# awslabs/flowgger

Hardware: NVIDIA H100
Metric: log lines/sec parsed (RFC5424) (higher is better)
Workload: dtype u8

## Files before the change

### flowgger_b200/csrc/fg_abi.cu

```cuda
#include <cuda_runtime.h>

#include <algorithm>
#include <chrono>
#include <cstdio>
#include <cstdlib>
#include <cstring>
#include <ctime>
#include <mutex>
#include <new>
#include <string>
#include <utility>
#include <vector>

#include "../../include/flowgger_cuda.h"
#include "fg_kernels.cuh"
#include "fg_status.h"
#include "fg_rfc3164.cuh"
#include "fg_tz.h"

namespace {

const char* kErrorStrings[FG_ST_COUNT] = {};
struct ErrorTableInit {
    ErrorTableInit() {
// ... 89 lines not shown
struct Handle {
    H h = nullptr;
    Handle() = default;
    Handle(Handle&& o) noexcept : h(o.h) { o.h = nullptr; }
    Handle(const Handle&) = delete;
    Handle& operator=(const Handle&) = delete;
    ~Handle() {
        if (h) destroy(h);
    }
    operator H() const { return h; }
};
using Event = Handle<cudaEvent_t>;
using Stream = Handle<cudaStream_t>;

struct StepEvents {
    Event h2d;
    Event k0, k1;
    Event cnt;
};

enum { T_ENTRIES, T_E8, T_ARENA, T_WIDE, T_COUNT };
struct TableShape {
    size_t width[3];
    size_t round;
};
constexpr TableShape kTableShape[T_COUNT] = {
    {{sizeof(fg_span), sizeof(uint64_t), 1}, 256},
    {{sizeof(uint64_t), 0, 0}, 256},
    {{1, 0, 0}, 256},
    {{sizeof(fg_wide_row), 0, 0}, 1},
};
static_assert(sizeof(fg_span) == sizeof(int2) && sizeof(fg_wide_row) == sizeof(fg::WideRow), "pinned rows mirror the device rows");
struct Table {
    Buf<uint8_t> col[3];
    size_t cap = 0;
};

struct TableUse {
    int table, counter;
    size_t div, floor;
    bool grow;
};
struct FormatTables {
    int n;
    TableUse use[4];
    const TableUse* begin() const { return use; }
    const TableUse* end() const { return use + n; }
};
constexpr FormatTables kFormatTables[4] = {
    {4, {{T_E8, fg::K5_ENTRIES, 24, 4096, false}, {T_ARENA, fg::K5_ARENA, 64, 64 << 10, false},
         {T_WIDE, fg::K5_WIDE_ROWS, 0, 1024, false}, {T_ENTRIES, fg::K5_WIDE_ENTRIES, 0, 4096, false}}},
    {1, {{T_ENTRIES, fg::K5_ENTRIES, 24, 4096, true}}},
    {1, {{T_ENTRIES, fg::K5_ENTRIES, 24, 4096, true}}},
    {2, {{T_ARENA, fg::K5_ARENA, 32, 64 << 10, false}, {T_ENTRIES, -1, 0, 256, false}}},
};

}

struct fg_ctx {
    int device = 0;
    size_t max_bytes = 0;
    int max_lines = 0;
    int chunk_lines = 0;
    Stream s_h2d, s_comp, s_d2h;
    Stream s_parse;
    Event ev_a, ev_b;
    Event ev_dom0, ev_dom1;
    Event ev_s0, ev_s1;
    std::vector<StepEvents> steps;
    std::vector<Event> ev_split;
    Event bounce_ev[2];
    Buf<uint8_t> bounce[2];
    Buf<uint32_t> counts;
    Buf<uint8_t> bytes;
    Buf<int32_t> offsets;
    Buf<uint32_t> k;
    Buf<uint8_t> flush;
    Table tab[T_COUNT];
    Buf<uint8_t> rows;
    Buf<int2> tmp_name;
    Buf<unsigned long long> tmp_val;
    Buf<uint8_t> tmp_meta;
    Buf<fg::Row5424, fg_row5424> rows5;
    Buf<uint32_t> esc_list, wide_list;
    Buf<uint32_t> enc_lens, enc_rel;
    Buf<unsigned long long> enc_base;
    Buf<uint8_t> enc_out;
    size_t enc_out_cap = 0;
    Buf<long long, int64_t> enc_offsets;
    Buf<uint8_t> enc_status;
    Buf<uint8_t> scan_temp;
    size_t scan_temp_bytes = 0;
    Buf<uint8_t> static_blob;
    int n_static = 0;
    const int32_t* d_static_key_off = nullptr;
    const int32_t* d_static_lit_off = nullptr;
    const int32_t* d_static_kind = nullptr;
    std::vector<std::pair<std::string, std::string>> gelf_extra;
    Buf<uint32_t> seg;
    Buf<int32_t> n_lines;
    Buf<uint8_t> invalid;
    Buf<int32_t> split_offsets;
    Buf<int32_t> cum;
    float last_split_ms = 0.f;
    int r3164_year = 0;
    int call_year = 1970;
    std::string tzdir;
    fg::TzHostTable tz_host;
    Buf<uint8_t> tz_blob;
    fg::TzDeviceTable tz_dev{};
    Buf<uint8_t> ltsv_blob;
    fg::LtsvDeviceConfig ltsv{};
    float last_dom_ms = 0.f;
    int res_n = 0;
    size_t res_bytes = 0;
    int res_fmt = -1;
    uint32_t res_tot[fg::K5_COUNT] = {};
    std::string last_error;
    int64_t launches = 0;
    int max_tile5 = 0;
    int num_sms = 0;
};

namespace {

constexpr int kColW[9] = {8, 4, 8, 8, 8, 8, 8, 8, 8};
enum { C_TS = 0, C_META, C_HOST, C_APP, C_PROC, C_MSGID, C_MSG, C_FULL, C_SD, C_COUNT };
size_t col_off(const fg_ctx* c, int col) {
    const size_t n = (size_t)c->max_lines;
    size_t o = 0;
    for (int k = 0; k < col; ++k) o += (size_t)kColW[k] * n;
    return o;
}

int fail(fg_ctx* c, int code, const char* what, cudaError_t e = cudaSuccess) {
    if (c) {
        c->last_error = what;
        if (e != cudaSuccess) {
            c->last_error += ": ";
            c->last_error += cudaGetErrorString(e);
        }
    }
    return code;
}

#define FG_CUDA(ctx, call)                                         \
    do {                                                           \
        cudaError_t _e = (call);                                   \
        if (_e != cudaSuccess) return fail(ctx, FG_E_CUDA, #call, _e); \
    } while (0)

cudaError_t create(Event& e, unsigned flags) { return cudaEventCreateWithFlags(&e.h, flags); }
cudaError_t create(Stream& s) { return cudaStreamCreateWithFlags(&s.h, cudaStreamNonBlocking); }

template <class T>
T* dev(const fg_ctx* c, int t, int col = 0) {
    return reinterpret_cast<T*>(c->tab[t].col[col].d);
}
template <class T>
T* host(const fg_ctx* c, int t, int col = 0) {
    return reinterpret_cast<T*>(c->tab[t].col[col].h);
}
uint32_t cap32(const fg_ctx* c, int t) { return (uint32_t)std::min<size_t>(c->tab[t].cap, 0xFFFFFFFFu); }

int grow_table(fg_ctx* c, int t, size_t rows) {
    const TableShape& S = kTableShape[t];
    Table& T = c->tab[t];
// ... 36 lines not shown
    std::vector<uint8_t> bytes;
    template <class V>
    size_t add(const V& v) {
        const size_t at = bytes.size();
        const uint8_t* src = reinterpret_cast<const uint8_t*>(v.data());
        bytes.insert(bytes.end(), src, src + v.size() * sizeof(v[0]));
        bytes.resize((bytes.size() + 15) & ~(size_t)15, 0);
        return at;
    }
    int upload(fg_ctx* c, Buf<uint8_t>& blob) {
        bytes.resize(bytes.size() + 16, 0);
        FG_CUDA(c, blob.alloc(bytes.size(), DEV));
        FG_CUDA(c, cudaMemcpy(blob.d, bytes.data(), bytes.size(), cudaMemcpyHostToDevice));
        return FG_OK;
    }
};

int upload_tz(fg_ctx* c) {
    const fg::TzHostTable& H = c->tz_host;
    Packer p;
    const size_t o_hash = p.add(H.hash), o_key = p.add(H.key), o_zone = p.add(H.zone), o_noff = p.add(H.name_off),
                 o_first = p.add(H.first), o_off = p.add(H.off), o_names = p.add(H.names);
    if (int rc = p.upload(c, c->tz_blob)) return rc;
    const uint8_t* b = c->tz_blob.d;
    fg::TzDeviceTable& T = c->tz_dev;
    T = H.view();
    T.hash = (const unsigned long long*)(b + o_hash);
    T.key = (const long long*)(b + o_key);
    T.zone = (const int32_t*)(b + o_zone);
    T.name_off = (const int32_t*)(b + o_noff);
    T.first = (const int32_t*)(b + o_first);
    T.off = (const int32_t*)(b + o_off);
    T.names = b + o_names;
    return FG_OK;
}

int upload_ltsv_config(fg_ctx* c, const fg_config* cfg) {
    std::vector<uint8_t> names, suffix;
    std::vector<int32_t> name_off{0}, types;
    const int ns = (cfg->ltsv_schema_names && cfg->ltsv_schema_types) ? cfg->ltsv_schema_len : 0;
    for (int k = 0; k < ns; ++k) {
        const char* s = cfg->ltsv_schema_names[k];
        names.insert(names.end(), (const uint8_t*)s, (const uint8_t*)s + strlen(s));
        name_off.push_back((int32_t)names.size());
        types.push_back(cfg->ltsv_schema_types[k]);
    }
    fg::LtsvDeviceConfig& L = c->ltsv;
    L.has_schema = (cfg->ltsv_has_schema || ns > 0) ? 1 : 0;
    L.n_schema = ns;
    L.suffix_present = 0;
    L.suffix_off[0] = 0;
    for (int t = 0; t < 5; ++t) {
        const char* s = cfg->ltsv_suffix[t];
        if (t > 0 && s) {
            L.suffix_present |= 1u << t;
            suffix.insert(suffix.end(), (const uint8_t*)s, (const uint8_t*)s + strlen(s));
        }
        L.suffix_off[t + 1] = (int32_t)suffix.size();
    }
    Packer p;
    const size_t o_names = p.add(names), o_off = p.add(name_off), o_types = p.add(types), o_suf = p.add(suffix);
    if (int rc = p.upload(c, c->ltsv_blob)) return rc;
    const uint8_t* b = c->ltsv_blob.d;
    L.names = b + o_names;
    L.name_off = (const int32_t*)(b + o_off);
    L.types = (const int32_t*)(b + o_types);
    L.suffix = b + o_suf;
    return FG_OK;
}

int current_year(const fg_ctx* c) {
    if (c->r3164_year != 0) return c->r3164_year;
    const time_t now = time(nullptr);
    struct tm g;
    gmtime_r(&now, &g);
    return g.tm_year + 1900;
}

int ensure_format(fg_ctx* c, int fmt) {
    const size_t L = (size_t)c->max_lines;
    if (fmt == FG_FMT_RFC5424) {
        if (!c->rows5.d) {
            FG_CUDA(c, c->rows5.alloc(L, BOTH));
            FG_CUDA(c, c->esc_list.alloc(L, DEV));
            FG_CUDA(c, c->wide_list.alloc(L, DEV));
        }
    } else if (!c->rows.d) {
        FG_CUDA(c, c->rows.alloc(col_off(c, C_COUNT), BOTH));
    }
    if (fmt == FG_FMT_GELF && !c->wide_list.d) FG_CUDA(c, c->wide_list.alloc(L, DEV));
    for (const TableUse& u : kFormatTables[fmt]) {
        const size_t first = u.div ? std::max<size_t>(c->max_bytes / u.div, u.floor) : u.floor;
        const size_t cap = c->tab[u.table].cap;
        if (u.grow ? cap < first : !cap)
            if (int rc = grow_table(c, u.table, first)) return rc;
    }
    if (fmt == FG_FMT_RFC3164) {
        if (!c->tz_host.loaded) {
            std::string err;
            if (!fg::tz_load_dir(c->tzdir.empty() ? nullptr : c->tzdir.c_str(), c->tz_host, err)) return fail(c, FG_E_ARG, err.c_str());
        }
        if (!c->tz_blob.d)
            if (int rc = upload_tz(c)) return rc;
    }
    if (fmt == FG_FMT_LTSV || fmt == FG_FMT_GELF) {
        const size_t need = (fmt == FG_FMT_LTSV ? c->max_bytes / 2 + L : c->max_bytes / 3) + 64;
        if (c->tmp_meta.n < need) {
            c->tmp_name.reset(); c->tmp_val.reset(); c->tmp_meta.reset();
            FG_CUDA(c, c->tmp_name.alloc(need, DEV));
            FG_CUDA(c, c->tmp_val.alloc(need, DEV));
            FG_CUDA(c, c->tmp_meta.alloc(need, DEV));
        }
    }
    return FG_OK;
}

int begin_call(fg_ctx* c, fg_format fmt) {
    if ((int)fmt < 0 || (int)fmt > 3) return fail(c, FG_E_ARG, "unknown format");
    FG_CUDA(c, cudaSetDevice(c->device));
    if (int rc = ensure_format(c, (int)fmt)) return rc;
    c->call_year = current_year(c);
    return FG_OK;
}

int pick_tile(const fg_ctx* c, size_t total_bytes, int n, int fmt) {
    const double mean = n > 0 ? (double)total_bytes / n : 0.0;
    const long lines = fg::lines_per_cta(fmt), gran = 8 * lines;
    const int max_tile[4] = {c->max_tile5, fg::kLtsvMaxTile, fg::kGelfMaxTile, fg::kR3164MaxTile};
    long t = (long)(mean * lines * 1.02) + gran;
    t = (t + gran - 1) / gran * gran;
    t = std::max(t, 8L * 1024);
    t = std::min(t, (long)max_tile[fmt]);
    return (int)t;
}

int launch_lines(fg_ctx* c, int fmt, int line0, int n, int tile, const uint8_t* invalid, int strip_eol, cudaStream_t s,
                 bool time_dominant = false) {
    if (fmt == FG_FMT_RFC5424) {
        fg::Parse5424Params P;
        P.bytes = c->bytes.d;
        P.offsets = c->offsets.d + line0;
        P.n = n;
        P.tile_bytes = tile;
        P.rows = reinterpret_cast<uint4*>(c->rows5.d + line0);
        P.entries = dev<unsigned long long>(c, T_E8);
        P.entry_cap = cap32(c, T_E8);
        P.counters = c->k.d;
        P.esc_list = c->esc_list.d;
        P.wide_list = c->wide_list.d;
        P.arena = dev<uint8_t>(c, T_ARENA);
        P.arena_cap = cap32(c, T_ARENA);
        P.wide_rows = dev<fg::WideRow>(c, T_WIDE);
        P.wide_cap = cap32(c, T_WIDE);
        P.wentry_name = dev<int2>(c, T_ENTRIES, 0);
        P.wentry_val = dev<unsigned long long>(c, T_ENTRIES, 1);
        P.wentry_meta = dev<uint8_t>(c, T_ENTRIES, 2);
        P.wentry_cap = cap32(c, T_ENTRIES);
        P.line0 = line0;
        P.bad_offsets = c->k.d + fg::K5_BAD_OFFSETS;
        P.line_invalid = invalid;
        P.strip_eol = strip_eol;
        P.num_sms = c->num_sms;
        FG_CUDA(c, cudaMemsetAsync(c->k.d + fg::K5_ESC_LIST, 0, 8, s));
        FG_CUDA(c, fg::launch_parse5424(P, s, time_dominant ? c->ev_dom0.h : nullptr, time_dominant ? c->ev_dom1.h : nullptr));
        c->launches += 2;
        return FG_OK;
    }
    fg::ParseParams P;
    P.bytes = c->bytes.d;
    P.offsets = c->offsets.d + line0;
    P.n = n;
    P.line0 = line0;
    P.tile_bytes = tile;
    P.num_sms = c->num_sms;
    uint8_t* r = c->rows.d;
    P.ts = (double*)(r + col_off(c, C_TS)) + line0;
    P.meta = (uint32_t*)(r + col_off(c, C_META)) + line0;
    P.host = (int2*)(r + col_off(c, C_HOST)) + line0;
    P.app = (int2*)(r + col_off(c, C_APP)) + line0;
    P.proc = (int2*)(r + col_off(c, C_PROC)) + line0;
    P.msgid = (int2*)(r + col_off(c, C_MSGID)) + line0;
    P.msg = (int2*)(r + col_off(c, C_MSG)) + line0;
    P.full = (int2*)(r + col_off(c, C_FULL)) + line0;
    P.sd = (int2*)(r + col_off(c, C_SD)) + line0;
    P.entry_name = dev<int2>(c, T_ENTRIES, 0);
    P.entry_val = dev<unsigned long long>(c, T_ENTRIES, 1);
    P.entry_meta = dev<uint8_t>(c, T_ENTRIES, 2);
    P.tmp_name = c->tmp_name.d;
    P.tmp_val = c->tmp_val.d;
    P.tmp_meta = c->tmp_meta.d;
    P.line_invalid = invalid;
    P.strip_eol = strip_eol;
    P.entry_counter = c->k.d + fg::K5_ENTRIES;
    P.entry_cap = cap32(c, T_ENTRIES);
    P.bad_offsets = c->k.d + fg::K5_BAD_OFFSETS;
    P.slow_list = c->wide_list.d;
    P.slow_count = c->k.d + fg::K5_WIDE_LIST;
    if (fmt == FG_FMT_GELF) FG_CUDA(c, cudaMemsetAsync(c->k.d + fg::K5_WIDE_LIST, 0, 4, s));
    P.ltsv = c->ltsv;
    P.r3164.year = c->call_year;
    P.r3164.tz = c->tz_dev;
    P.r3164.arena = dev<uint8_t>(c, T_ARENA);
    P.r3164.arena_cap = cap32(c, T_ARENA);
    P.r3164.arena_counter = c->k.d + fg::K5_ARENA;
    if (time_dominant) FG_CUDA(c, cudaEventRecord(c->ev_dom0, s));
    FG_CUDA(c, fg::launch_parse(fmt, P, s));
    if (time_dominant) FG_CUDA(c, cudaEventRecord(c->ev_dom1, s));
    c->launches += fmt == FG_FMT_GELF ? 2 : 1;
    return FG_OK;
}

int launch_encode(fg_ctx* c, int k, int l0, int n, int tile, cudaStream_t s) {
    fg::GelfEncodeParams E;
    E.bytes = c->bytes.d;
    E.offsets = c->offsets.d + l0;
    E.n = n;
    E.rows = reinterpret_cast<const uint4*>(c->rows5.d + l0);
    E.entries = dev<unsigned long long>(c, T_E8);
    E.arena = dev<uint8_t>(c, T_ARENA);
    E.wide_rows = dev<fg::WideRow>(c, T_WIDE);
    E.wentry_name = dev<int2>(c, T_ENTRIES, 0);
    E.wentry_val = dev<unsigned long long>(c, T_ENTRIES, 1);
    E.wentry_meta = dev<uint8_t>(c, T_ENTRIES, 2);
    E.static_blob = c->static_blob.d;
    E.n_static = c->n_static;
    E.static_key_off = c->d_static_key_off;
    E.static_lit_off = c->d_static_lit_off;
    E.static_kind = c->d_static_kind;
    E.lens = c->enc_lens.d + l0;
    E.rel = c->enc_rel.d + l0;
    E.base = c->enc_base.d + k;
    E.out = c->enc_out.d;
    E.out_cap = c->enc_out_cap;
    E.out_offsets = c->enc_offsets.d + l0;
    E.status = c->enc_status.d + l0;
    E.bad_offsets = c->k.d + fg::K5_BAD_OFFSETS;
    E.entry_cap = cap32(c, T_E8);
    E.wide_cap = cap32(c, T_WIDE);
    E.wentry_cap = cap32(c, T_ENTRIES);
    E.tile_bytes = std::min(4 * tile, c->max_tile5);
    FG_CUDA(c, fg::launch_gelf_encode(E, c->scan_temp.d, c->scan_temp_bytes, s));
    c->launches += 4;
    return FG_OK;
}

bool col_used(int col) { return !(col == C_APP || col == C_PROC || col == C_MSGID); }
// ... 754 lines not shown
```

### flowgger_b200/csrc/fg_kernels.cuh

```cuda
#pragma once
#include <stdint.h>
#ifdef FG_HOST_EMU
#include "../../tests/emu/cuda_shim.h"
#else
#include <cuda_runtime.h>
#endif

namespace fg {

struct LtsvDeviceConfig {
    int32_t has_schema;
    int32_t n_schema;
    const uint8_t* names;
    const int32_t* name_off;
    const int32_t* types;
    const uint8_t* suffix;
    int32_t suffix_off[6];
    uint32_t suffix_present;
};

struct TzDeviceTable {
    int32_t n_names;
    int32_t min_len, max_len;
    uint32_t first_mask[8];
    const unsigned long long* hash;
    const int32_t* zone;
    const int32_t* name_off;
    const uint8_t* names;
    const int32_t* first;
    const long long* key;
    const int32_t* off;
};
struct R3164DeviceConfig {
    int32_t year;
    TzDeviceTable tz;
    uint8_t* arena;
    uint32_t arena_cap;
    uint32_t* arena_counter;
};

struct ParseParams {
    const uint8_t* bytes;
    const int32_t* offsets;
    int32_t n;
    int32_t line0;
    int32_t tile_bytes;
    double* ts;
    uint32_t* meta;
    int2* host;
    int2* app;
    int2* proc;
    int2* msgid;
    int2* msg;
    int2* full;
    int2* sd;
    int2* entry_name;
    unsigned long long* entry_val;
    uint8_t* entry_meta;
    int2* tmp_name;
    unsigned long long* tmp_val;
    uint8_t* tmp_meta;
    const uint8_t* line_invalid;
    int32_t strip_eol;
    uint32_t* entry_counter;
    uint32_t entry_cap;
    const uint32_t* bad_offsets;
    uint32_t* slow_list;
    uint32_t* slow_count;
    int32_t num_sms;
    LtsvDeviceConfig ltsv;
    R3164DeviceConfig r3164;
};

struct Row5424 {
    double ts;
    uint32_t meta;
    uint32_t sd_first;
    uint16_t sd_count;
    uint16_t sp[5];
    uint16_t msg_off, msg_len;
};
static_assert(sizeof(Row5424) == 32, "Row5424 must be 32 bytes");
struct WideRow {
    int32_t line;
    uint32_t meta;
    double ts;
    int2 host, app, proc, msgid, msg, full, sd;
};
static_assert(sizeof(WideRow) == 72, "WideRow must be 72 bytes");

enum { K5_ENTRIES = 0, K5_ARENA = 1, K5_WIDE_ROWS = 2, K5_WIDE_ENTRIES = 3, K5_ESC_LIST = 4, K5_WIDE_LIST = 5, K5_BAD_OFFSETS = 6,
       K5_COUNT = 8 };

struct Parse5424Params {
    const uint8_t* bytes;
    const int32_t* offsets;
    int32_t n;
    int32_t tile_bytes;
    uint4* rows;
    unsigned long long* entries;
    uint32_t entry_cap;
    uint32_t* counters;
    uint32_t* esc_list;
    uint32_t* wide_list;
    uint8_t* arena;
    uint32_t arena_cap;
    WideRow* wide_rows;
    uint32_t wide_cap;
    int2* wentry_name;
    unsigned long long* wentry_val;
    uint8_t* wentry_meta;
    uint32_t wentry_cap;
    int32_t line0;
    const uint32_t* bad_offsets;
    const uint8_t* line_invalid;
    int32_t strip_eol;
    int32_t num_sms;
};

cudaError_t launch_parse5424(const Parse5424Params& p, cudaStream_t stream, cudaEvent_t dom0 = nullptr, cudaEvent_t dom1 = nullptr);
cudaError_t configure_parse5424(int max_tile_bytes);
int parse5424_smem_bytes(int tile_bytes);

struct GelfEncodeParams {
    const uint8_t* bytes;
    const int32_t* offsets;
    int32_t n;
    const uint4* rows;
    const unsigned long long* entries;
    const uint8_t* arena;
    const WideRow* wide_rows;
    const int2* wentry_name;
    const unsigned long long* wentry_val;
    const uint8_t* wentry_meta;
    const uint8_t* static_blob;
    int32_t n_static;
    const int32_t* static_key_off;
    const int32_t* static_lit_off;
    const int32_t* static_kind;
    uint32_t* lens;
    uint32_t* rel;
    unsigned long long* base;
    uint8_t* out;
    unsigned long long out_cap;
    long long* out_offsets;
    uint8_t* status;
    const uint32_t* bad_offsets;
    uint32_t entry_cap, wide_cap, wentry_cap;
    int32_t tile_bytes;
};
cudaError_t configure_gelf_encode(int max_tile_bytes);
cudaError_t launch_gelf_encode(const GelfEncodeParams& p, void* d_scan_temp, size_t scan_temp_bytes, cudaStream_t stream);
size_t gelf_scan_temp_bytes(int n);

#ifndef FG_R5_LINES
#define FG_R5_LINES 64
#endif
#ifndef FG_R5_MINB
#define FG_R5_MINB 16
#endif
constexpr int kRfc5424LinesPerCta = FG_R5_LINES;
constexpr int kRfc5424CtasPerSm = FG_R5_MINB;
#ifndef FG_LTSV_LINES
#define FG_LTSV_LINES 64
#endif
#ifndef FG_LTSV_THREADS
#define FG_LTSV_THREADS 256
#endif
constexpr int kLtsvLinesPerCta = FG_LTSV_LINES;
constexpr int kLtsvThreadsPerCta = FG_LTSV_THREADS;
constexpr int kLtsvStageSlots = kLtsvLinesPerCta * 24;
constexpr int kLtsvMaxTile = 65024;
#ifndef FG_GELF_LINES
#define FG_GELF_LINES 64
#endif
#ifndef FG_GELF_THREADS
#define FG_GELF_THREADS 256
#endif
constexpr int kGelfLinesPerCta = FG_GELF_LINES;
constexpr int kGelfThreadsPerCta = FG_GELF_THREADS;
constexpr int kGelfCtasPerSm = 3;
constexpr int kGelfStageSlots = kGelfLinesPerCta * 16;
constexpr int kGelfMaxTile = 65024;
#ifndef FG_R3_LINES
#define FG_R3_LINES 64
#endif
// ... 33 lines not shown
```

### flowgger_b200/csrc/fg_parse5424.cu

```cuda
#include "fg_kernels.cuh"

#include "fg_common.cuh"
#include "fg_r5fast.cuh"
#include "fg_rfc5424.cuh"
#include "fg_status.h"
#include "fg_tma.cuh"

namespace fg {

namespace {

constexpr int kFastLines = kRfc5424LinesPerCta;
constexpr int kFastCtasPerSm = kRfc5424CtasPerSm;

template <int LINES, int MINB>
__global__ void __launch_bounds__(LINES, MINB) parse5424_kernel(const __grid_constant__ Parse5424Params P) {
    extern __shared__ __align__(128) uint8_t tile[];
    __shared__ __align__(8) uint64_t mbar;
    __shared__ uint32_t scan_ws[2 * (LINES / 32)];
    __shared__ uint32_t s_base[3];

    const int tid = threadIdx.x;
    const uint32_t lane = (uint32_t)tid & 31u;
    const int first = blockIdx.x * LINES;
    const int last = min(P.n, first + LINES);
    uint32_t* bmI = reinterpret_cast<uint32_t*>(tile + P.tile_bytes);
    if (*P.bad_offsets) return;
    if (tid == 0) mbar_init(&mbar, 1);
    __syncthreads();

    uint32_t parity = 0;
    int cur = first;
    while (cur < last) {
        const int i = cur + tid;
        const int o0 = __ldg(P.offsets + min(i, last));
        const int o1 = __ldg(P.offsets + min(i + 1, last));
        const int ocur = __ldg(P.offsets + cur);
        const int base = ocur & ~15;
        const bool fits = (i < last) && (o1 - base <= P.tile_bytes);
        const int r = __syncthreads_count(fits);
        if (r == 0) {
            if (tid == 0) P.wide_list[atomicAdd(P.counters + K5_WIDE_LIST, 1u)] = (uint32_t)cur;
            cur += 1;
            continue;
        }
        const int oend = __ldg(P.offsets + cur + r);
        const uint32_t nbytes = (uint32_t)((oend - base) + 15) & ~15u;
        if (tid == 0) {
            fence_proxy_async();
            mbar_expect_tx(&mbar, nbytes);
            bulk_g2s(tile, P.bytes + base, nbytes, &mbar);
        }
        mbar_wait(&mbar, parity);
        parity ^= 1u;

        const int nword = (int)((nbytes + 31u) >> 5);
        for (int g = tid; g < nword; g += LINES) {
            const uint4 v0 = reinterpret_cast<const uint4*>(tile)[2 * g], v1 = reinterpret_cast<const uint4*>(tile)[2 * g + 1];
            bmI[g] = r5_classify16(v0.x, v0.y, v0.z, v0.w) | (r5_classify16(v1.x, v1.y, v1.z, v1.w) << 16);
        }
        if (tid < 3) bmI[nword + tid] = 0;
        __syncthreads();

        const bool active = tid < r;
        int ls = active ? o0 - base : 0;
        int le = active ? o1 - base : 0;
        bool bad_utf8 = false;
        if (P.strip_eol && le > ls) {
            if (P.strip_eol == 2) {
                if (tile[le - 1] == 0) --le;
            } else if (tile[le - 1] == '\n') {
                --le;
                if (le > ls && tile[le - 1] == '\r') --le;
            }
            if (P.line_invalid != nullptr && P.line_invalid[i]) bad_utf8 = true;
        }
        const bool too_long = le - ls > 65535;
        R5Fast res;
        const bool regular = r5_regular(tile, bmI, ls, (too_long || bad_utf8 || !active) ? ls : le, res);
        if (bad_utf8) {
            res.status = FG_ES_INVALID_UTF8;
            res.n_entries = 0;
        }
        const bool wide = active && !regular && !bad_utf8;
        const uint32_t my_n = (active && !wide && res.status == FG_ST_OK) ? res.n_entries : 0u;
        const bool esc = my_n != 0u && res.esc;

        uint32_t xa = my_n, xb = (esc ? 1u : 0u) | (wide ? 0x100u : 0u);
#pragma unroll
        for (int d = 1; d < 32; d <<= 1) {
            const uint32_t ya = __shfl_up_sync(0xFFFFFFFFu, xa, d), yb = __shfl_up_sync(0xFFFFFFFFu, xb, d);
            if (lane >= (uint32_t)d) { xa += ya; xb += yb; }
        }
        const int wid = tid >> 5;
        constexpr int kWarps = LINES / 32;
        if (lane == 31u) { scan_ws[wid] = xa; scan_ws[kWarps + wid] = xb; }
        __syncthreads();
        uint32_t before_a = 0, before_b = 0, total = 0, total_b = 0;
#pragma unroll
        for (int w = 0; w < kWarps; ++w) {
            const uint32_t ta = scan_ws[w], tb = scan_ws[kWarps + w];
            if (w < wid) { before_a += ta; before_b += tb; }
            total += ta;
            total_b += tb;
        }
        const uint32_t excl = before_a + xa - my_n;
        const uint32_t pos_b = before_b + xb - ((esc ? 1u : 0u) | (wide ? 0x100u : 0u));
        const uint32_t n_esc = total_b & 0xFFu, n_wide = total_b >> 8;
        if (total | total_b) {
            if (tid == 0 && total) s_base[0] = atomicAdd(P.counters + K5_ENTRIES, total);
            if (tid == 32 % LINES && n_esc) s_base[1] = atomicAdd(P.counters + K5_ESC_LIST, n_esc);
            if (tid == 33 % LINES && n_wide) s_base[2] = atomicAdd(P.counters + K5_WIDE_LIST, n_wide);
            __syncthreads();
        }
        const uint32_t esc_at = pos_b & 0xFFu, wide_at = pos_b >> 8;
        uint32_t my_begin = 0;
        if (my_n) {
            my_begin = s_base[0] + excl;
            if ((unsigned long long)my_begin + my_n <= (unsigned long long)P.entry_cap) {
                unsigned long long* dst = P.entries + my_begin;
                for (uint32_t k = 0; k < my_n; ++k) dst[k] = res.stage[k];
            }
        }
        if (esc) P.esc_list[s_base[1] + esc_at] = (uint32_t)i;
        if (wide) P.wide_list[s_base[2] + wide_at] = (uint32_t)i;
        if (active && !wide) {
            const bool ok = res.status == FG_ST_OK;
            const uint32_t meta = ok ? (res.facility << 8) | (res.severity << 16) | (res.flags << 24) : res.status | 0x00FFFF00u;
            uint4 lo4, hi4;
            lo4.x = (uint32_t)__double2loint(res.ts);
            lo4.y = (uint32_t)__double2hiint(res.ts);
            lo4.z = meta;
            lo4.w = my_begin;
            hi4.x = my_n | ((uint32_t)res.sp1 << 16);
            hi4.y = (uint32_t)res.sp2 | ((uint32_t)res.sp3 << 16);
            hi4.z = (uint32_t)res.sp4 | ((uint32_t)res.sp5 << 16);
            hi4.w = (uint32_t)res.msg_o | ((uint32_t)res.msg_l << 16);
            if (!ok) {
                lo4.x = lo4.y = 0u;
                hi4 = make_uint4(0u, 0u, 0u, 0u);
            }
            P.rows[2 * (size_t)i] = lo4;
            P.rows[2 * (size_t)i + 1] = hi4;
        }
        __syncthreads();
        cur += r;
    }
}

__device__ __forceinline__ void unescape_lines(const Parse5424Params& P, uint32_t first_item, uint32_t stride) {
    const uint32_t cnt = P.counters[K5_ESC_LIST];
    const uint32_t lane = threadIdx.x & 31u;
    for (uint32_t j0 = first_item; j0 < cnt; j0 += stride) {
        const uint32_t j = j0 + lane;
        const bool valid = j < cnt;
        uint32_t first = 0, count = 0;
        int o0 = 0;
        if (valid) {
            const uint32_t line = P.esc_list[j];
            const uint4 lo4 = P.rows[2 * (size_t)line], hi4 = P.rows[2 * (size_t)line + 1];
            o0 = P.offsets[line];
            first = lo4.w;
            count = hi4.x & 0xFFFFu;
            if ((unsigned long long)first + count > (unsigned long long)P.entry_cap) count = 0;
        }
        uint32_t need = 0;
        for (uint32_t e = 0; e < count; ++e) {
            const unsigned long long v = P.entries[first + e];
            if (!(v & kE8Header) && (v & kE8Esc)) need += (2u + (uint32_t)((v >> 32) & 0xFFFFu) - ((uint32_t)((v >> 16) & 0xFFFFu) + 2u) + 1u) & ~1u;
        }
        uint32_t inc = need;
#pragma unroll
        for (int d = 1; d < 32; d <<= 1) {
            const uint32_t y = __shfl_up_sync(0xFFFFFFFFu, inc, d);
            if (lane >= (uint32_t)d) inc += y;
        }
        const uint32_t warp_total = __shfl_sync(0xFFFFFFFFu, inc, 31);
        uint32_t abase = 0;
        if (lane == 0 && warp_total) abase = atomicAdd(P.counters + K5_ARENA, warp_total);
        abase = __shfl_sync(0xFFFFFFFFu, abase, 0);
        if ((unsigned long long)abase + warp_total > (unsigned long long)P.arena_cap) continue;
        uint32_t at = abase + inc - need;
        uint32_t e = 0;
        for (;;) {
            unsigned long long v = 0;
            bool have = false;
            for (; e < count; ++e) {
                v = P.entries[first + e];
                if (!(v & kE8Header) && (v & kE8Esc)) { have = true; break; }
            }
            if (!__any_sync(0xFFFFFFFFu, have)) break;
            const int ne = (int)((v >> 16) & 0xFFFFu), ve = (int)((v >> 32) & 0xFFFFu);
            const int len = have ? ve - (ne + 2) : 0;
            const uint8_t* src = P.bytes + o0 + ne + 2;
            uint8_t* dst = P.arena + at + 2;
            int k = 0, o = 0;
            while (__any_sync(0xFFFFFFFFu, k < len)) {
                if (k < len) {
                    const uint32_t c = src[k++];
                    if (c != '\\') {
                        dst[o++] = (uint8_t)c;
                    } else if (k < len) {
                        const uint32_t d = src[k++];
                        if (d != '"' && d != '\\' && d != ']') dst[o++] = '\\';
                        dst[o++] = (uint8_t)d;
                    }
                }
            }
            if (have) {
                *reinterpret_cast<uint16_t*>(P.arena + at) = (uint16_t)o;
                P.entries[first + e] = (v & 0xFFFFFFFFull) | ((unsigned long long)(at >> 1) << 32) | kE8Arena;
                at += (2u + (uint32_t)len + 1u) & ~1u;
                ++e;
            }
        }
    }
}

__device__ __forceinline__ void wide_lines(const Parse5424Params& P, int (*marks)[32], uint32_t first_item, uint32_t stride) {
    const uint32_t cnt = P.counters[K5_WIDE_LIST];
    const uint32_t lane = threadIdx.x & 31u;
    const EntrySink sink = {P.wentry_name, P.wentry_val, P.wentry_meta};
    for (uint32_t j0 = first_item; j0 < cnt; j0 += stride) {
        const uint32_t j = j0 + lane;
        const bool valid = j < cnt;
        uint32_t line = 0;
        int o0 = 0, len = 0;
        bool bad_utf8 = false;
        if (valid) {
            line = P.wide_list[j];
            o0 = P.offsets[line];
            len = P.offsets[line + 1] - o0;
            if (P.strip_eol && len > 0) {
                if (P.strip_eol == 2) {
                    if (P.bytes[o0 + len - 1] == 0) --len;
                } else if (P.bytes[o0 + len - 1] == '\n') {
                    --len;
                    if (len > 0 && P.bytes[o0 + len - 1] == '\r') --len;
                }
                if (P.line_invalid != nullptr && P.line_invalid[line]) bad_utf8 = true;
            }
            if (bad_utf8) len = 0;
        }
        LineResult res;
        rfc5424_parse_line<32>(P.bytes + o0, len, o0, &marks[0][lane], res, sink, 0u, false);
        uint32_t n = (valid && !bad_utf8 && res.status == FG_ST_OK) ? res.n_entries : 0u;
        uint32_t wbase = 0;
        if (n) {
            wbase = atomicAdd(P.counters + K5_WIDE_ENTRIES, n);
            if ((unsigned long long)wbase + n > (unsigned long long)P.wentry_cap) n = 0;
        }
        {
            LineResult again;
            rfc5424_parse_line<32>(P.bytes + o0, n ? len : 0, o0, &marks[0][lane], again, sink, wbase, true);
        }
        if (!valid) continue;
        for (uint32_t k = 0; k < n; ++k) {
            const uint32_t e = wbase + k;
            const uint8_t m = sink.meta[e];
            if ((m & 0x07u) == 0u && (m & 0x08u)) {
                const unsigned long long v = sink.val[e];
                const uint32_t off = (uint32_t)v, l = (uint32_t)(v >> 32);
                const uint32_t ul = (uint32_t)r5_unescape(P.bytes + off, (int)l, nullptr);
                const uint32_t at = atomicAdd(P.counters + K5_ARENA, (ul + 1u) & ~1u);
                if ((unsigned long long)at + ul <= (unsigned long long)P.arena_cap) r5_unescape(P.bytes + off, (int)l, P.arena + at);
                sink.val[e] = (unsigned long long)at | ((unsigned long long)ul << 32);
                sink.meta[e] = (uint8_t)0x80u;
            }
        }
        if (bad_utf8) {
            res.status = FG_ES_INVALID_UTF8;
            res.flags = 0;
            res.facility = res.severity = 0xFFu;
        }
        const bool ok = res.status == FG_ST_OK;
        if (!ok) {
            P.rows[2 * (size_t)line] = make_uint4(0u, 0u, res.status | 0x00FFFF00u, 0u);
            P.rows[2 * (size_t)line + 1] = make_uint4(0u, 0u, 0u, 0u);
            continue;
        }
        const uint32_t widx = atomicAdd(P.counters + K5_WIDE_ROWS, 1u);
        const uint32_t meta = res.status | (res.facility << 8) | (res.severity << 16) | ((res.flags | kFlagWide) << 24);
        if (widx < P.wide_cap) {
            WideRow w;
            w.line = P.line0 + (int32_t)line;
            w.meta = meta;
            w.ts = res.ts;
            w.host = make_int2(ok ? o0 + res.host_o : -1, res.host_l);
            w.app = make_int2(ok ? o0 + res.app_o : -1, res.app_l);
            w.proc = make_int2(ok ? o0 + res.proc_o : -1, res.proc_l);
            w.msgid = make_int2(ok ? o0 + res.mid_o : -1, res.mid_l);
            w.msg = make_int2(ok && res.msg_o >= 0 ? o0 + res.msg_o : -1, res.msg_l);
            w.full = make_int2(ok && res.full_o >= 0 ? o0 + res.full_o : -1, res.full_l);
            w.sd = make_int2((int)wbase, (int)(ok ? n : 0u));
            P.wide_rows[widx] = w;
        }
        P.rows[2 * (size_t)line] = make_uint4((uint32_t)__double2loint(res.ts), (uint32_t)__double2hiint(res.ts), meta, widx);
        P.rows[2 * (size_t)line + 1] = make_uint4(0u, 0u, 0u, 0u);
    }
}

__global__ void __launch_bounds__(128) post5424_kernel(const __grid_constant__ Parse5424Params P, int esc_ctas) {
    __shared__ int marks[4][6][32];
    if (*P.bad_offsets) return;
    const uint32_t warp = threadIdx.x >> 5;
    if ((int)blockIdx.x < esc_ctas) {
        unescape_lines(P, (blockIdx.x * 4u + warp) * 32u, (uint32_t)esc_ctas * 128u);
    } else {
        const uint32_t wctas = gridDim.x - (uint32_t)esc_ctas;
        wide_lines(P, marks[warp], ((blockIdx.x - (uint32_t)esc_ctas) * 4u + warp) * 32u, wctas * 128u);
    }
}

}

int parse5424_smem_bytes(int tile_bytes) { return tile_bytes + tile_bytes / 8 + 16; }

cudaError_t configure_parse5424(int max_tile_bytes) {
    return cudaFuncSetAttribute(parse5424_kernel<kFastLines, kFastCtasPerSm>, cudaFuncAttributeMaxDynamicSharedMemorySize,
                                parse5424_smem_bytes(max_tile_bytes));
}

cudaError_t launch_parse5424(const Parse5424Params& p, cudaStream_t stream, cudaEvent_t dom0, cudaEvent_t dom1) {
    if (p.n <= 0) return cudaSuccess;
    const int grid = (p.n + kFastLines - 1) / kFastLines;
    if (dom0) cudaEventRecord(dom0, stream);
    parse5424_kernel<kFastLines, kFastCtasPerSm><<<grid, kFastLines, parse5424_smem_bytes(p.tile_bytes), stream>>>(p);
    if (dom1) cudaEventRecord(dom1, stream);
    const long long sms = p.num_sms;
    const int esc_ctas = (int)min((long long)(p.n + 127) / 128, sms * 12);
    const int wide_ctas = (int)min((long long)(p.n + 127) / 128, sms * 4);
    post5424_kernel<<<esc_ctas + wide_ctas, 128, 0, stream>>>(p, esc_ctas);
    return cudaGetLastError();
}

}
```

### flowgger_b200/csrc/fg_r5fast.cuh

```cuda
#pragma once
#include "fg_common.cuh"
#include "fg_status.h"

namespace fg {

FG_DEV uint32_t r5_flags(uint32_t w) {
    const uint32_t low = w & 0x7F7F7F7Fu;
    const uint32_t a2 = low + 0x5D5D5D5Du;
    const uint32_t a1 = low + 0x01010101u;
    const uint32_t x = (w & 0x1E1E1E1Eu) ^ 0x1C1C1C1Cu;
    const uint32_t a3 = x + 0x7F7F7F7Fu;
    return (~a2 | a1 | w | ~a3) & 0x80808080u;
}
FG_DEV uint32_t r5_nibble_top(uint32_t f) { return f * 0x00204081u; }
FG_DEV uint32_t r5_gather16(uint32_t f0, uint32_t f1, uint32_t f2, uint32_t f3) {
    const uint32_t n0 = r5_nibble_top(f0), n1 = r5_nibble_top(f1), n2 = r5_nibble_top(f2), n3 = r5_nibble_top(f3);
    return (n0 >> 28) | ((n1 >> 24) & 0xF0u) | ((n2 >> 20) & 0xF00u) | ((n3 >> 16) & 0xF000u);
}
FG_DEV uint32_t r5_classify16(uint32_t w0, uint32_t w1, uint32_t w2, uint32_t w3) {
    return r5_gather16(r5_flags(w0), r5_flags(w1), r5_flags(w2), r5_flags(w3));
}
FG_DEV uint32_t r5_window(const uint32_t* bm, int t) {
    const int k = t >> 5;
    return fg_funnel_r(bm[k], bm[k + 1], (uint32_t)t & 31u);
}

constexpr unsigned long long kE8Esc = 1ull << 48;
constexpr unsigned long long kE8Header = 1ull << 63;
constexpr unsigned long long kE8Arena = 1ull << 62;
FG_DEV unsigned long long r5_pack_pair8(int ns, int ne, int ve, bool esc) {
    return (unsigned long long)(uint32_t)ns | ((unsigned long long)(uint32_t)ne << 16) | ((unsigned long long)(uint32_t)ve << 32) |
           (esc ? kE8Esc : 0ull);
}
FG_DEV unsigned long long r5_pack_header8(int es, int id_end, uint32_t pairs) {
    return (unsigned long long)(uint32_t)es | ((unsigned long long)(uint32_t)id_end << 16) | ((unsigned long long)(pairs & 0xFFFFu) << 32) | kE8Header;
}

struct R5Fast {
    double ts;
    uint32_t status, facility, severity, flags;
    int sp1, sp2, sp3, sp4, sp5;
    int msg_o, msg_l;
    uint32_t n_entries;
    unsigned long long* stage;
    bool esc;
};

FG_DEV int r5_unescape(const uint8_t* v, int len, uint8_t* out) {
    int o = 0;
    bool esc = false;
    for (int k = 0; k < len; ++k) {
        const uint8_t c = v[k];
        if (!esc) {
            if (c == '\\') esc = true;
            else {
                if (out) out[o] = c;
                ++o;
            }
        } else {
            if (c != '"' && c != '\\' && c != ']') {
                if (out) out[o] = '\\';
                ++o;
            }
            if (out) out[o] = c;
            ++o;
            esc = false;
        }
    }
    return o;
}

FG_DEV int r5_unescape_to(const uint8_t* v, int len, uint8_t* out) {
    int o = 0;
    for (int k = 0; k < len; ++k) {
        const uint32_t c = v[k];
        if (c != '\\') {
            out[o++] = (uint8_t)c;
        } else if (k + 1 < len) {
            const uint32_t d = v[++k];
            if (d != '"' && d != '\\' && d != ']') out[o++] = '\\';
            out[o++] = (uint8_t)d;
        }
    }
    return o;
}

constexpr uint32_t kFlagWide = 0x80u;

FG_DEV uint32_t r5_digit(const uint8_t* T, int at, uint32_t& worst) {
    const uint32_t d = (uint32_t)T[at] - (uint32_t)'0';
    worst = max(worst, d);
    return d;
}

FG_DEV bool r5_regular(uint8_t* T, const uint32_t* bmI, int ls, int le, R5Fast& r) {
    r.ts = 0.0;
    r.status = FG_ST_OK;
    r.facility = 0xFFu;
    r.severity = 0xFFu;
    r.flags = 0;
    r.sp1 = r.sp2 = r.sp3 = r.sp4 = r.sp5 = 0;
    r.msg_o = r.msg_l = 0;
    r.n_entries = 0;
    r.stage = nullptr;
    r.esc = false;
    bool ok = le - ls >= 32;

    int sp[6];
    {
        int t = ls + 1;
#pragma unroll
        for (int k = 0; k < 6; ++k) {
            uint32_t W = r5_window(bmI, t);
            if (k == 1 && W == 0u) {
                t += 32;
                W = r5_window(bmI, t);
            }
            t += fg_ffs(W) - 1;
            ok = ok && W != 0u && t < le && T[t] == ' ';
            sp[k] = t;
            t = ok ? t + 1 : ls;
        }
    }
    uint32_t bad = 0;
    {
        const int l0 = sp[0] - ls;
        ok = ok && T[ls] == '<' && l0 >= 4 && l0 <= 6;
        const int gt = ok ? sp[0] - 2 : ls;
        ok = ok && T[gt] == '>' && T[gt + 1] == '1';
        uint32_t pri = 0;
        for (int q = ls + 1; q < gt; ++q) pri = pri * 10u + r5_digit(T, q, bad);
        ok = ok && pri <= 255u;
        r.facility = pri >> 3;
        r.severity = pri & 7u;
    }
    {
        const int a = ok ? sp[0] + 1 : ls, e = ok ? sp[1] : ls;
        const int L = e - a;
        ok = ok && L >= 20;
        const int z = ok ? e - 1 : ls;
        const bool zulu = T[z] == 'Z';
        const int zone = zulu ? z : z - 5;
        DateTime t;
        t.year = (int)(r5_digit(T, a, bad) * 1000u + r5_digit(T, a + 1, bad) * 100u + r5_digit(T, a + 2, bad) * 10u + r5_digit(T, a + 3, bad));
        t.month = (int)(r5_digit(T, a + 5, bad) * 10u + r5_digit(T, a + 6, bad));
        t.day = (int)(r5_digit(T, a + 8, bad) * 10u + r5_digit(T, a + 9, bad));
        t.hour = (int)(r5_digit(T, a + 11, bad) * 10u + r5_digit(T, a + 12, bad));
        t.minute = (int)(r5_digit(T, a + 14, bad) * 10u + r5_digit(T, a + 15, bad));
        t.second = (int)(r5_digit(T, a + 17, bad) * 10u + r5_digit(T, a + 18, bad));
        ok = ok && T[a + 4] == '-' && T[a + 7] == '-' && T[a + 10] == 'T' && T[a + 13] == ':' && T[a + 16] == ':';
        const int fl = zone - (a + 19);
        ok = ok && (fl == 0 || (fl >= 2 && fl <= 10 && T[a + 19] == '.'));
        uint32_t nanos = 0, mult = 100000000u;
#pragma unroll
        for (int k = 0; k < 9; ++k) {
            if (k + 1 < fl) nanos += r5_digit(T, a + 20 + k, bad) * mult;
            mult /= 10u;
        }
        t.nanos = nanos;
        int off = 0;
        if (!zulu) {
            const uint32_t sg = T[zone];
            const int oh = (int)(r5_digit(T, zone + 1, bad) * 10u + r5_digit(T, zone + 2, bad));
            const int om = (int)(r5_digit(T, zone + 4, bad) * 10u + r5_digit(T, zone + 5, bad));
            ok = ok && (sg == '+' || sg == '-') && T[zone + 3] == ':' && oh <= 23 && om <= 59 && zone >= a + 19;
            off = oh * 3600 + om * 60;
            if (sg == '-') off = -off;
        }
        t.offset_seconds = off;
        ok = ok && bad <= 9u && t.second <= 59;
        if (!ok) { t.year = 2000; t.month = 1; t.day = 1; t.hour = t.minute = t.second = 0; t.nanos = 0; t.offset_seconds = 0; }
        double ts = 0.0;
        ok = finish_datetime(t, false, ts) && ok;
        r.ts = ts;
    }
    fg_syncwarp();

    const int d = ok ? sp[5] + 1 : ls;
    int msg_from = le;
    bool walk = false;
    ok = ok && d < le;
    if (ok) {
        const uint32_t c0 = T[d];
        if (c0 == '-') msg_from = d + 1;
        else if (c0 == '[') walk = true;
        else ok = false;
    }
    {
        const int sbase = (ls + 7) & ~7;
        unsigned long long* stg = (unsigned long long*)(T + sbase);
        uint32_t n = 0, pairs = 0, hdr = 0;
        int i = d + 1, elem_start = 0, id_end = 0;
        bool st_id = true, active = walk, any_esc = false;
        while (fg_any(active)) {
            if (active && st_id) {
                const uint32_t W = r5_window(bmI, i);
                const int s1 = i + fg_ffs(W) - 1;
                if (W == 0u || s1 >= le || T[s1] != ' ') { ok = false; active = false; }
                else { elem_start = i; id_end = s1; i = s1 + 1; st_id = false; hdr = n++; pairs = 0; }
            }
            int e = i;
            if (active) {
                const uint32_t W = r5_window(bmI, i);
                e = i + fg_ffs(W) - 1;
                if (W == 0u || (W & 1u) || e + 2 >= le || T[e] != '=' || T[e + 1] != '"') { ok = false; active = false; }
            }
            int c = e + 2;
            bool has_bs = false;
            {
                bool s = active;
                for (;;) {
                    if (s) {
                        uint32_t W = r5_window(bmI, c);
                        const int room = le - c;
                        if (room < 32) W &= (1u << room) - 1u;
                        int adv = 32;
                        while (W) {
                            const int b = fg_ffs(W) - 1;
                            const uint32_t ch = T[c + b];
                            if (ch == '"') { adv = b; s = false; break; }
                            W &= W - 1u;
                            if (ch == '\\') {
                                has_bs = true;
                                W &= ~(2u << b);
                                if (b == 31) adv = 33;
                            }
                        }
                        c += adv;
                        if (s && c >= le) { c = le; s = false; }
                    }
                    if (!fg_any(s)) break;
                }
            }
            if (active) {
                if (c + 1 >= le || sbase + 8 * ((int)n + 1) > c + 1) { ok = false; active = false; }
                else {
                    stg[n++] = r5_pack_pair8(i - ls, e - ls, c - ls, has_bs);
                    any_esc |= has_bs;
                    ++pairs;
                    const uint32_t nx = T[c + 1];
                    if (nx == ' ') {
                        i = c + 2;
                        if (i >= le) { ok = false; active = false; }
                    } else if (nx == ']') {
                        stg[hdr] = r5_pack_header8(elem_start - ls, id_end - ls, pairs);
                        const uint32_t n2 = c + 2 < le ? T[c + 2] : 0u;
                        if (n2 == ' ') { msg_from = c + 2; active = false; }
                        else if (n2 == '[') { i = c + 3; st_id = true; }
                        else { ok = false; active = false; }
                    } else { ok = false; active = false; }
                }
            }
        }
        if (walk && ok) {
            r.n_entries = n;
            r.stage = stg;
            r.esc = any_esc;
        }
    }

    int hi = le, lo = msg_from;
    {
        bool plain_end = true, plain_start = true;
        if (ok) {
            const uint32_t cl = T[le - 1];
            plain_end = cl > 0x20u && cl < 0x80u;
            plain_start = false;
            if (msg_from + 1 < le) {
                const uint32_t c0 = T[msg_from], c1 = T[msg_from + 1];
                plain_start = c0 == ' ' && c1 > 0x20u && c1 < 0x80u;
            }
        }
        if (fg_any(!plain_end)) {
            if (ok && !plain_end) hi = trim_end(T, msg_from, le);
        }
        if (fg_any(!plain_start)) {
            if (ok) lo = plain_start ? msg_from + 1 : trim_start(T, msg_from, hi);
        } else {
            lo = msg_from + 1;
        }
    }
    if (ok) {
        if (hi > lo) {
            r.msg_o = lo - ls;
            r.msg_l = hi - lo;
        } else {
            r.msg_o = msg_from - ls;
            r.msg_l = 0;
        }
        r.sp1 = sp[1] - ls;
        r.sp2 = sp[2] - ls;
        r.sp3 = sp[3] - ls;
        r.sp4 = sp[4] - ls;
        r.sp5 = sp[5] - ls;
    }
    fg_syncwarp();
    return ok;
}

}
```

Measured before the change: 6.730 billion.

## Fuse structured-data unescaping into RFC5424 parse kernel, drop esc_list post pass

Moves the unescaping of backslash-escaped structured-data values out of the separate post5424 pass and into the main parse kernel. Each line now computes its arena byte need while walking the SD section, a warp scan reserves arena space in a single atomic per block, and a warp-cooperative ballot-based unescaper writes values straight from the shared tile or global bytes. This removes the esc_list buffer, one counter reset, the extra post-kernel CTAs, and the re-reads of rows and entries from global memory. In exchange the parse kernel gains extra registers and warp-synchronous loops, which may reduce occupancy on the main hot path.

```diff
diff --git a/flowgger_b200/csrc/fg_abi.cu b/flowgger_b200/csrc/fg_abi.cu
--- a/flowgger_b200/csrc/fg_abi.cu
+++ b/flowgger_b200/csrc/fg_abi.cu
@@ -195,7 +195,7 @@
     Buf<unsigned long long> tmp_val;
     Buf<uint8_t> tmp_meta;
     Buf<fg::Row5424, fg_row5424> rows5;
-    Buf<uint32_t> esc_list, wide_list;
+    Buf<uint32_t> wide_list;
     Buf<uint32_t> enc_lens, enc_rel;
     Buf<unsigned long long> enc_base;
     Buf<uint8_t> enc_out;
@@ -398,7 +398,6 @@
     if (fmt == FG_FMT_RFC5424) {
         if (!c->rows5.d) {
             FG_CUDA(c, c->rows5.alloc(L, BOTH));
-            FG_CUDA(c, c->esc_list.alloc(L, DEV));
             FG_CUDA(c, c->wide_list.alloc(L, DEV));
         }
     } else if (!c->rows.d) {
@@ -462,7 +461,6 @@
         P.entries = dev<unsigned long long>(c, T_E8);
         P.entry_cap = cap32(c, T_E8);
         P.counters = c->k.d;
-        P.esc_list = c->esc_list.d;
         P.wide_list = c->wide_list.d;
         P.arena = dev<uint8_t>(c, T_ARENA);
         P.arena_cap = cap32(c, T_ARENA);
@@ -477,7 +475,7 @@
         P.line_invalid = invalid;
         P.strip_eol = strip_eol;
         P.num_sms = c->num_sms;
-        FG_CUDA(c, cudaMemsetAsync(c->k.d + fg::K5_ESC_LIST, 0, 8, s));
+        FG_CUDA(c, cudaMemsetAsync(c->k.d + fg::K5_WIDE_LIST, 0, 4, s));
         FG_CUDA(c, fg::launch_parse5424(P, s, time_dominant ? c->ev_dom0.h : nullptr, time_dominant ? c->ev_dom1.h : nullptr));
         c->launches += 2;
         return FG_OK;
diff --git a/flowgger_b200/csrc/fg_kernels.cuh b/flowgger_b200/csrc/fg_kernels.cuh
--- a/flowgger_b200/csrc/fg_kernels.cuh
+++ b/flowgger_b200/csrc/fg_kernels.cuh
@@ -89,8 +89,7 @@
 };
 static_assert(sizeof(WideRow) == 72, "WideRow must be 72 bytes");
 
-enum { K5_ENTRIES = 0, K5_ARENA = 1, K5_WIDE_ROWS = 2, K5_WIDE_ENTRIES = 3, K5_ESC_LIST = 4, K5_WIDE_LIST = 5, K5_BAD_OFFSETS = 6,
-       K5_COUNT = 8 };
+enum { K5_ENTRIES = 0, K5_ARENA = 1, K5_WIDE_ROWS = 2, K5_WIDE_ENTRIES = 3, K5_WIDE_LIST = 5, K5_BAD_OFFSETS = 6, K5_COUNT = 8 };
 
 struct Parse5424Params {
     const uint8_t* bytes;
@@ -101,7 +100,6 @@
     unsigned long long* entries;
     uint32_t entry_cap;
     uint32_t* counters;
-    uint32_t* esc_list;
     uint32_t* wide_list;
     uint8_t* arena;
     uint32_t arena_cap;
diff --git a/flowgger_b200/csrc/fg_parse5424.cu b/flowgger_b200/csrc/fg_parse5424.cu
--- a/flowgger_b200/csrc/fg_parse5424.cu
+++ b/flowgger_b200/csrc/fg_parse5424.cu
@@ -12,6 +12,21 @@
 
 constexpr int kFastLines = kRfc5424LinesPerCta;
 constexpr int kFastCtasPerSm = kRfc5424CtasPerSm;
+
+__device__ __forceinline__ int unescape_warp(const uint8_t* src, int len, uint8_t* out, uint32_t lane) {
+    uint32_t carry = 0;
+    int o = 0;
+    for (int c0 = 0; c0 < len; c0 += 32) {
+        const int j = c0 + (int)lane;
+        const uint32_t b = j < len ? src[j] : 0u, nb = j + 1 < len ? src[j + 1] : 0u;
+        const uint32_t bs = __ballot_sync(0xFFFFFFFFu, b == '\\');
+        const uint32_t sp = __ballot_sync(0xFFFFFFFFu, j + 1 >= len || nb == '"' || nb == '\\' || nb == ']');
+        const uint32_t keep = r5_unescape_keep(bs, sp, carry) & (len - c0 >= 32 ? 0xFFFFFFFFu : (1u << (len - c0)) - 1u);
+        if ((keep >> lane) & 1u) out[o + __popc(keep & ((1u << lane) - 1u))] = (uint8_t)b;
+        o += __popc(keep);
+    }
+    return o;
+}
 
 template <int LINES, int MINB>
 __global__ void __launch_bounds__(LINES, MINB) parse5424_kernel(const __grid_constant__ Parse5424Params P) {
@@ -84,9 +99,9 @@
         }
         const bool wide = active && !regular && !bad_utf8;
         const uint32_t my_n = (active && !wide && res.status == FG_ST_OK) ? res.n_entries : 0u;
-        const bool esc = my_n != 0u && res.esc;
-
-        uint32_t xa = my_n, xb = (esc ? 1u : 0u) | (wide ? 0x100u : 0u);
+        const uint32_t need = my_n ? res.arena_need : 0u;
+
+        uint32_t xa = my_n, xb = need | (wide ? 0x1000000u : 0u);
 #pragma unroll
         for (int d = 1; d < 32; d <<= 1) {
             const uint32_t ya = __shfl_up_sync(0xFFFFFFFFu, xa, d), yb = __shfl_up_sync(0xFFFFFFFFu, xb, d);
@@ -105,24 +120,42 @@
             total_b += tb;
         }
         const uint32_t excl = before_a + xa - my_n;
-        const uint32_t pos_b = before_b + xb - ((esc ? 1u : 0u) | (wide ? 0x100u : 0u));
-        const uint32_t n_esc = total_b & 0xFFu, n_wide = total_b >> 8;
+        const uint32_t pos_b = before_b + xb - (need | (wide ? 0x1000000u : 0u));
+        const uint32_t n_arena = total_b & 0xFFFFFFu, n_wide = total_b >> 24;
         if (total | total_b) {
             if (tid == 0 && total) s_base[0] = atomicAdd(P.counters + K5_ENTRIES, total);
-            if (tid == 32 % LINES && n_esc) s_base[1] = atomicAdd(P.counters + K5_ESC_LIST, n_esc);
+            if (tid == 32 % LINES && n_arena) s_base[1] = atomicAdd(P.counters + K5_ARENA, n_arena);
             if (tid == 33 % LINES && n_wide) s_base[2] = atomicAdd(P.counters + K5_WIDE_LIST, n_wide);
             __syncthreads();
         }
-        const uint32_t esc_at = pos_b & 0xFFu, wide_at = pos_b >> 8;
-        uint32_t my_begin = 0;
-        if (my_n) {
-            my_begin = s_base[0] + excl;
-            if ((unsigned long long)my_begin + my_n <= (unsigned long long)P.entry_cap) {
-                unsigned long long* dst = P.entries + my_begin;
-                for (uint32_t k = 0; k < my_n; ++k) dst[k] = res.stage[k];
-            }
-        }
-        if (esc) P.esc_list[s_base[1] + esc_at] = (uint32_t)i;
+        const uint32_t arena_at = pos_b & 0xFFFFFFu, wide_at = pos_b >> 24;
+        const uint32_t my_begin = my_n ? s_base[0] + excl : 0u;
+        const uint32_t n_out = (unsigned long long)my_begin + my_n <= (unsigned long long)P.entry_cap ? my_n : 0u;
+        const bool unescape = need && (unsigned long long)s_base[1] + n_arena <= (unsigned long long)P.arena_cap;
+        const int stage_end = n_out ? (int)(reinterpret_cast<const uint8_t*>(res.stage + n_out) - tile) : 0;
+        uint32_t at = s_base[1] + arena_at;
+        for (uint32_t k = 0; fg_any(k < n_out); ++k) {
+            unsigned long long v = k < n_out ? res.stage[k] : 0ull;
+            const bool e = unescape && k < n_out && !(v & kE8Header) && (v & kE8Esc);
+            int vs = 0, len = 0;
+            const uint32_t rec = at;
+            if (e) {
+                vs = ls + (int)((v >> 16) & 0xFFFFu) + 2;
+                len = r5_row_value_len(v);
+                v = r5_arena_row(v, at);
+                at += r5_arena_bytes(len);
+            }
+            if (k < n_out) P.entries[my_begin + k] = v;
+            for (uint32_t m = __ballot_sync(0xFFFFFFFFu, e); m; m &= m - 1u) {
+                const int src = __ffs((int)m) - 1;
+                const int s_vs = __shfl_sync(0xFFFFFFFFu, vs, src), s_len = __shfl_sync(0xFFFFFFFFu, len, src);
+                const uint32_t s_at = __shfl_sync(0xFFFFFFFFu, rec, src);
+                const bool covered = s_vs < __shfl_sync(0xFFFFFFFFu, stage_end, src);
+                uint8_t* out = P.arena + s_at + 2;
+                const int o = covered ? unescape_warp(P.bytes + base + s_vs, s_len, out, lane) : unescape_warp(tile + s_vs, s_len, out, lane);
+                if (lane == (uint32_t)src) *reinterpret_cast<uint16_t*>(P.arena + s_at) = (uint16_t)o;
+            }
+        }
         if (wide) P.wide_list[s_base[2] + wide_at] = (uint32_t)i;
         if (active && !wide) {
             const bool ok = res.status == FG_ST_OK;
@@ -145,75 +178,6 @@
         }
         __syncthreads();
         cur += r;
-    }
-}
-
-__device__ __forceinline__ void unescape_lines(const Parse5424Params& P, uint32_t first_item, uint32_t stride) {
-    const uint32_t cnt = P.counters[K5_ESC_LIST];
-    const uint32_t lane = threadIdx.x & 31u;
-    for (uint32_t j0 = first_item; j0 < cnt; j0 += stride) {
-        const uint32_t j = j0 + lane;
-        const bool valid = j < cnt;
-        uint32_t first = 0, count = 0;
-        int o0 = 0;
-        if (valid) {
-            const uint32_t line = P.esc_list[j];
-            const uint4 lo4 = P.rows[2 * (size_t)line], hi4 = P.rows[2 * (size_t)line + 1];
-            o0 = P.offsets[line];
-            first = lo4.w;
-            count = hi4.x & 0xFFFFu;
-            if ((unsigned long long)first + count > (unsigned long long)P.entry_cap) count = 0;
-        }
-        uint32_t need = 0;
-        for (uint32_t e = 0; e < count; ++e) {
-            const unsigned long long v = P.entries[first + e];
-            if (!(v & kE8Header) && (v & kE8Esc)) need += (2u + (uint32_t)((v >> 32) & 0xFFFFu) - ((uint32_t)((v >> 16) & 0xFFFFu) + 2u) + 1u) & ~1u;
-        }
-        uint32_t inc = need;
-#pragma unroll
-        for (int d = 1; d < 32; d <<= 1) {
-            const uint32_t y = __shfl_up_sync(0xFFFFFFFFu, inc, d);
-            if (lane >= (uint32_t)d) inc += y;
-        }
-        const uint32_t warp_total = __shfl_sync(0xFFFFFFFFu, inc, 31);
-        uint32_t abase = 0;
-        if (lane == 0 && warp_total) abase = atomicAdd(P.counters + K5_ARENA, warp_total);
-        abase = __shfl_sync(0xFFFFFFFFu, abase, 0);
-        if ((unsigned long long)abase + warp_total > (unsigned long long)P.arena_cap) continue;
-        uint32_t at = abase + inc - need;
-        uint32_t e = 0;
-        for (;;) {
-            unsigned long long v = 0;
-            bool have = false;
-            for (; e < count; ++e) {
-                v = P.entries[first + e];
-                if (!(v & kE8Header) && (v & kE8Esc)) { have = true; break; }
-            }
-            if (!__any_sync(0xFFFFFFFFu, have)) break;
-            const int ne = (int)((v >> 16) & 0xFFFFu), ve = (int)((v >> 32) & 0xFFFFu);
-            const int len = have ? ve - (ne + 2) : 0;
-            const uint8_t* src = P.bytes + o0 + ne + 2;
-            uint8_t* dst = P.arena + at + 2;
-            int k = 0, o = 0;
-            while (__any_sync(0xFFFFFFFFu, k < len)) {
-                if (k < len) {
-                    const uint32_t c = src[k++];
-                    if (c != '\\') {
-                        dst[o++] = (uint8_t)c;
-                    } else if (k < len) {
-                        const uint32_t d = src[k++];
-                        if (d != '"' && d != '\\' && d != ']') dst[o++] = '\\';
-                        dst[o++] = (uint8_t)d;
-                    }
-                }
-            }
-            if (have) {
-                *reinterpret_cast<uint16_t*>(P.arena + at) = (uint16_t)o;
-                P.entries[first + e] = (v & 0xFFFFFFFFull) | ((unsigned long long)(at >> 1) << 32) | kE8Arena;
-                at += (2u + (uint32_t)len + 1u) & ~1u;
-                ++e;
-            }
-        }
     }
 }
 
@@ -300,16 +264,11 @@
     }
 }
 
-__global__ void __launch_bounds__(128) post5424_kernel(const __grid_constant__ Parse5424Params P, int esc_ctas) {
+__global__ void __launch_bounds__(128) post5424_kernel(const __grid_constant__ Parse5424Params P) {
     __shared__ int marks[4][6][32];
     if (*P.bad_offsets) return;
     const uint32_t warp = threadIdx.x >> 5;
-    if ((int)blockIdx.x < esc_ctas) {
-        unescape_lines(P, (blockIdx.x * 4u + warp) * 32u, (uint32_t)esc_ctas * 128u);
-    } else {
-        const uint32_t wctas = gridDim.x - (uint32_t)esc_ctas;
-        wide_lines(P, marks[warp], ((blockIdx.x - (uint32_t)esc_ctas) * 4u + warp) * 32u, wctas * 128u);
-    }
+    wide_lines(P, marks[warp], (blockIdx.x * 4u + warp) * 32u, gridDim.x * 128u);
 }
 
 }
@@ -328,9 +287,8 @@
     parse5424_kernel<kFastLines, kFastCtasPerSm><<<grid, kFastLines, parse5424_smem_bytes(p.tile_bytes), stream>>>(p);
     if (dom1) cudaEventRecord(dom1, stream);
     const long long sms = p.num_sms;
-    const int esc_ctas = (int)min((long long)(p.n + 127) / 128, sms * 12);
     const int wide_ctas = (int)min((long long)(p.n + 127) / 128, sms * 4);
-    post5424_kernel<<<esc_ctas + wide_ctas, 128, 0, stream>>>(p, esc_ctas);
+    post5424_kernel<<<wide_ctas, 128, 0, stream>>>(p);
     return cudaGetLastError();
 }
 
diff --git a/flowgger_b200/csrc/fg_r5fast.cuh b/flowgger_b200/csrc/fg_r5fast.cuh
--- a/flowgger_b200/csrc/fg_r5fast.cuh
+++ b/flowgger_b200/csrc/fg_r5fast.cuh
@@ -43,6 +43,7 @@
     int msg_o, msg_l;
     uint32_t n_entries;
     unsigned long long* stage;
+    uint32_t arena_need;
     bool esc;
 };
 
@@ -85,6 +86,23 @@
     return o;
 }
 
+FG_DEV uint32_t r5_arena_bytes(int len) { return (2u + (uint32_t)len + 1u) & ~1u; }
+
+FG_DEV unsigned long long r5_arena_row(unsigned long long v, uint32_t at) {
+    return (v & 0xFFFFFFFFull) | ((unsigned long long)(at >> 1) << 32) | kE8Arena;
+}
+FG_DEV uint32_t r5_unescape_keep(uint32_t bs, uint32_t sp, uint32_t& carry) {
+    const uint32_t b = bs & ~carry;
+    const uint32_t follows = (b << 1) | carry;
+    const uint32_t odd_starts = b & ~0x55555555u & ~follows;
+    const uint32_t sum = odd_starts + b;
+    const uint32_t escaped = (0x55555555u ^ (sum << 1)) & follows;
+    const uint32_t escaper = bs & ~escaped;
+    carry = escaper >> 31;
+    return ~(escaper & sp);
+}
+FG_DEV int r5_row_value_len(unsigned long long v) { return (int)((v >> 32) & 0xFFFFu) - ((int)((v >> 16) & 0xFFFFu) + 2); }
+
 constexpr uint32_t kFlagWide = 0x80u;
 
 FG_DEV uint32_t r5_digit(const uint8_t* T, int at, uint32_t& worst) {
@@ -103,6 +121,7 @@
     r.msg_o = r.msg_l = 0;
     r.n_entries = 0;
     r.stage = nullptr;
+    r.arena_need = 0;
     r.esc = false;
     bool ok = le - ls >= 32;
 
@@ -191,7 +210,8 @@
         unsigned long long* stg = (unsigned long long*)(T + sbase);
         uint32_t n = 0, pairs = 0, hdr = 0;
         int i = d + 1, elem_start = 0, id_end = 0;
-        bool st_id = true, active = walk, any_esc = false;
+        uint32_t need = 0;
+        bool st_id = true, active = walk;
         while (fg_any(active)) {
             if (active && st_id) {
                 const uint32_t W = r5_window(bmI, i);
@@ -236,7 +256,7 @@
                 if (c + 1 >= le || sbase + 8 * ((int)n + 1) > c + 1) { ok = false; active = false; }
                 else {
                     stg[n++] = r5_pack_pair8(i - ls, e - ls, c - ls, has_bs);
-                    any_esc |= has_bs;
+                    if (has_bs) need += r5_arena_bytes(c - (e + 2));
                     ++pairs;
                     const uint32_t nx = T[c + 1];
                     if (nx == ' ') {
@@ -255,7 +275,8 @@
         if (walk && ok) {
             r.n_entries = n;
             r.stage = stg;
-            r.esc = any_esc;
+            r.arena_need = need;
+            r.esc = need != 0u;
         }
     }
 
```

Result: faster. 6.889 billion, median of 6 (+2.4%).
